# liangxuy/ReGenNet

Measured on AMD Instinct MI355X. Metric: sampled motions/sec, higher is better.
Workload: dtype bf16 MFMA operands, fp32 accumulate/LayerNorm/softmax, for 990 of 1000 steps; fp16 MFMA operands for the next 8; split-bf16 (x3) for the last 2; 1 GPU; ntu: [B=256/GPU,56,6,60] online/concat/no_cond L8 d512, 1000-step DDPM, Philox noise, hipGraph=on; batch_per_gpu=256, global_batch=256, denoiser_evals_per_motion=1000, parallelism=batch-shard x1

## Files before the change

regennet_amd/csrc/rgn_layers.hip:

```cpp
#include "rgn_internal.h"
#include "rgn_device.h"
#include "rgn_tail.h"
#include "rgn_sampler.h"

#include <hip/hip_runtime.h>

#include <cmath>
#include <type_traits>
#include <utility>

namespace rgn {

#ifndef RGN_LY_ST_AUX
#define RGN_LY_ST_AUX 16
#endif

constexpr int LY_NTH = 512, LY_KB = 4096;
constexpr int LY_X = 0, LY_Y = 64 * 1024, LY_EXCH = LY_Y, LY_RED = 128 * 1024, LY_REDF = 2 * 8 * 64, LY_VEC = LY_RED + 2 * LY_REDF * 4, LY_VECW = 640,
              LY_LDS = 160 * 1024;
constexpr int LY_PF = LY_VEC + 8 * LY_VECW * 4;
static_assert(LY_PF + 8 * 256 <= LY_LDS, "LDS map");
enum { V_BO = 0, V_G1 = 64, V_G2 = 128, V_B2 = 192, V_SPV = 256, V_BF1 = 320 , V_BF2 = 448, V_G3 = 512, V_B3 = 576 };
constexpr int LY_RDA = 6;
constexpr int LY_RDM = 8;
struct LYT {
    static constexpr int MT = 2, NT = 2, NW = 8, R = 64, RD = LY_RDM, KB = LY_KB, RED = LY_RED, REDF = LY_REDF;
};

#ifdef RGN_LY_STAMPS
__device__ long long g_ly_st[1024][16];
#define RGN_LYT(i)                                                                                   \
    {                                                                                                \
        __builtin_amdgcn_sched_barrier(0);                                                           \
        if (threadIdx.x == 0 && blockIdx.x < 1024 && l == RGN_LY_STAMPS) g_ly_st[blockIdx.x][i] = __builtin_readcyclecounter(); \
        __builtin_amdgcn_sched_barrier(0);                                                           \
    }
#define RGN_LYS(i)                                                                                   \
    {                                                                                                \
        __builtin_amdgcn_sched_barrier(0);                                                           \
        if (threadIdx.x == 0 && blockIdx.x < 1024 && it == 1) g_ly_st[blockIdx.x][i] = __builtin_readcyclecounter(); \
        __builtin_amdgcn_sched_barrier(0);                                                           \
    }
#else
#define RGN_LYT(i)
#define RGN_LYS(i)
#endif

constexpr int LY_XLD = 356, LY_TILE = 0, LY_XIMG = 92160, LY_NKX = 11;
static_assert(64 * LY_XLD * 4 <= LY_XIMG && LY_XIMG + LY_NKX * 4096 <= LY_LDS, "step boundary LDS map");

template <bool STEPS, bool GUIDED = false, bool F16 = false, bool INPAINT = false>
__global__ __launch_bounds__(LY_NTH, 2) void k_layers(LayersArgs g) {
    static_assert(STEPS || !GUIDED, "guidance inside the launch needs the step boundary");
    static_assert(STEPS || !INPAINT, "in-painting (rgn_set_inpainting) belongs to the step boundary");
    using OP = OpFmt<F16>;
    using op_t = typename OP::t;
    using op8 = typename OP::v8;
    using op4 = typename OP::v4;
    extern __shared__ __attribute__((aligned(16))) char smem[];
    const int tid = threadIdx.x, lane = tid & 63;
    const int wave = __builtin_amdgcn_readfirstlane(tid >> 6);
    const int wn = wave & 3, hg = wave >> 2;
    const int l31 = lane & 31, kh = lane >> 5;
    const int b = xcd_affine(blockIdx.x, gridDim.x), Tq = g.Tq;
    const size_t row0 = (size_t)b * Tq;
#ifdef RGN_LY_PRIO
    if (wave >= 4) __builtin_amdgcn_s_setprio(RGN_LY_PRIO);
#endif
    float* vec = reinterpret_cast<float*>(smem + LY_VEC) + wave * LY_VECW;
    const int lane16 = lane * 16;
    tile_dma_in(smem + LY_X, g.h, g.rows, row0, Tq, lane, wave);
    const int first_step = (g.stepvec || STEPS) ? *g.d_step : 0;
    const TailLane tl = tail_lane<LYT>(smem, lane, wave);
    static_assert(LY_X == 0, "a_off addresses the image at byte 0");
    int a_off[2], a_offy[2];
    tail_a_off(a_off, lane);
    tail_a_off(a_offy, a_off, LY_Y);
    using Pass = TailPass;
    op8 wf[LY_RDM][2];
    const float qs2 = g.qscale * 1.44269504088896340736f;

    f32x4 qb[4];
    float vb1;
    auto load_qbias = [&](const float* bqkv, int r) {
        const float* bq = bqkv + (2 * r + hg) * 128 + wn * 32;
#pragma unroll
        for (int i4 = 0; i4 < 4; ++i4) qb[i4] = *reinterpret_cast<const f32x4*>(bq + 8 * i4 + 4 * kh);
        vb1 = bq[1024 + l31];
    };

    wait_vmcnt<0>();
    __builtin_amdgcn_s_barrier();
    load_qbias(g.lw[0].bqkv, 0);

    const int nit = STEPS ? g.steps : 1;
    auto out_proj = [&](f32x16 (&acc)[2][2], int wv) {
#pragma unroll
        for (int a2 = 0; a2 < 2; ++a2)
#pragma unroll
            for (int b2 = 0; b2 < 2; ++b2)
#pragma unroll
                for (int i = 0; i < 16; ++i) acc[a2][b2][i] = 0.f;
        if (wv < 6) {
            const int cb0 = 2 * wv;
            const Pass p_out{__builtin_amdgcn_make_buffer_rsrc(const_cast<__bf16*>(g.Wout) + (size_t)cb0 * 1024, 0, (16 * g.nb_out - cb0) * 2048, 0x00020000), LY_NKX * 2048, 0};
#pragma unroll
            for (int s2 = 0; s2 < LY_RDM - 1; ++s2) tail_load_g<OP, LYT>(wf, tl, p_out, s2, s2);
            tail_gemm<OP, LYT, 32, false, 0>(acc, wf, tl, a_off, p_out, p_out);
        }
    };
    for (int it = 0; it < nit; ++it) {
    const int step = first_step - it;
    for (int pass = 0; pass < (GUIDED ? 2 : 1); ++pass) {
    if (GUIDED && pass == 1) {
        f32x16 accp[2][2];
        int wave_p = wave, lane_p = lane, b_p = b;
        asm volatile("" : "+s"(wave_p), "+s"(b_p));
        asm volatile("" : "+v"(lane_p));
        out_proj(accp, wave_p);
        if (wave_p < 6) {
            float* pk = g.park + ((size_t)b_p * 6 + wave_p) * 4096 + lane_p * 4;
#pragma unroll
            for (int nt = 0; nt < 2; ++nt)
#pragma unroll
                for (int mt = 0; mt < 2; ++mt)
#pragma unroll
                    for (int i4 = 0; i4 < 4; ++i4)
                        *reinterpret_cast<f32x4*>(pk + ((nt * 2 + mt) * 4 + i4) * 256) = f32x4{accp[nt][mt][4 * i4], accp[nt][mt][4 * i4 + 1], accp[nt][mt][4 * i4 + 2], accp[nt][mt][4 * i4 + 3]};
        }
        __builtin_amdgcn_s_barrier();
        tile_dma_in<16>(smem + LY_X, g.h, g.rows, g.half + (size_t)b_p * Tq, Tq, lane_p, wave_p);
        wait_vmcnt<0>();
        __builtin_amdgcn_s_barrier();
    }
    for (int l = 0; l < g.L; ++l) {
        const LayerWts& w = g.lw[l];
        RGN_LYT(0)
        op4 attk[2][2][4];
        float bo_r = 0.f;
        {
            struct PassA { __amdgpu_buffer_rsrc_t rs; };
            auto qrs = [&](int r) {
                const int blk = (2 * r + hg) * 4 + wn;
                return __builtin_amdgcn_make_buffer_rsrc(const_cast<__bf16*>(w.Wqkv) + (size_t)blk * 1024, 0, 3 * 512 * 512 * 2 - blk * 2048, 0x00020000);
            };
            const PassA pa[2] = {{qrs(0)}, {qrs(1)}};
            op8 wq[LY_RDA][3];
            auto load_ga = [&](const PassA& ps, int hs, int slot) {
                int soff;
                asm volatile("s_mov_b32 %0, %1" : "=s"(soff) : "i"(frag_granule(hs, 48 * 2048)));
#pragma unroll
                for (int t = 0; t < 3; ++t)
                    wq[slot][t] = __builtin_bit_cast(op8, __builtin_amdgcn_raw_buffer_load_b128(ps.rs, lane16, soff + t * (16 * 2048), 0));
            };
            constexpr int AH = LY_RDA - 1;
#pragma unroll
            for (int s = 0; s < AH; ++s) load_ga(pa[0], s, s);
#pragma unroll
            for (int r = 0; r < 2; ++r) {
                const int head = 2 * r + hg;
                f32x16 acc[2][3];
#pragma unroll
                for (int ta = 0; ta < 2; ++ta)
#pragma unroll
                    for (int i4 = 0; i4 < 4; ++i4)
#pragma unroll
                        for (int e = 0; e < 4; ++e) {
                            acc[ta][0][4 * i4 + e] = qb[i4][e];
                            acc[ta][1][4 * i4 + e] = 0.f;
                            acc[ta][2][4 * i4 + e] = vb1;
                        }
                __builtin_amdgcn_sched_barrier(0);
                {
                    op8 af[2];
#pragma unroll
                    for (int ta = 0; ta < 2; ++ta) af[ta] = *reinterpret_cast<const op8*>(smem + a_off[0] + ta * 2048);
#pragma unroll
                    for (int hs = 0; hs < 32; ++hs) {
                        op8 afn[2];
#pragma unroll
                        for (int ta = 0; ta < 2; ++ta) {
                            afn[ta] = af[ta];
                            if (hs + 1 < 32) afn[ta] = *reinterpret_cast<const op8*>(smem + ((hs + 1) >> 1) * LY_KB + a_off[(hs + 1) & 1] + ta * 2048);
                        }
                        if (hs + AH < 32) load_ga(pa[r], hs + AH, (32 * r + hs + AH) % LY_RDA);
                        else if (r == 0) load_ga(pa[1], hs + AH - 32, (32 * r + hs + AH) % LY_RDA);
                        if (hs + AH < 32 || r == 0) {
                            if (hs < AH) wait_vmcnt<3 * AH + 5>();
                            else wait_vmcnt<3 * AH>();
                        }
                        const int slot = (32 * r + hs) % LY_RDA;
#pragma unroll
                        for (int t = 0; t < 3; ++t)
#pragma unroll
                            for (int ta = 0; ta < 2; ++ta) {
                                if (t < 2) acc[ta][t] = OP::mfma(wq[slot][t], af[ta], acc[ta][t]);
                                else acc[ta][t] = OP::mfma(af[ta], wq[slot][t], acc[ta][t]);
                            }
#pragma unroll
                        for (int ta = 0; ta < 2; ++ta) af[ta] = afn[ta];
                    }
                }
                __builtin_amdgcn_sched_barrier(0);
                RGN_LYT(1 + 3 * r)
                op8 qh[2][2], kf[2][2], vh[2][2];
#pragma unroll
                for (int ta = 0; ta < 2; ++ta)
#pragma unroll
                    for (int sl = 0; sl < 2; ++sl)
#pragma unroll
                        for (int j = 0; j < 8; ++j) {
                            const int i = 8 * sl + j;
                            qh[ta][sl][j] = (op_t)acc[ta][0][i];
                            kf[ta][sl][j] = (op_t)acc[ta][1][i];
                            vh[ta][sl][j] = (op_t)acc[ta][2][i];
                        }
                if (r == 0) load_qbias(w.bqkv, 1);
                else bo_r = w.bo[64 * wave + lane];
                f32x16 st[3];
#pragma unroll
                for (int tl = 0; tl < 3; ++tl) {
                    const int kj = tl >> 1, qtile = tl ? 1 : 0;
#pragma unroll
                    for (int i = 0; i < 16; ++i) st[tl][i] = 0.f;
#pragma unroll
                    for (int sl = 0; sl < 2; ++sl) st[tl] = OP::mfma(kf[kj][sl], qh[qtile][sl], st[tl]);
                }
                f32x4* sred = reinterpret_cast<f32x4*>(smem + LY_EXCH);
#pragma unroll
                for (int tl = 0; tl < 3; ++tl)
#pragma unroll
                    for (int i4 = 0; i4 < 4; ++i4) {
                        const f32x4 v = {st[tl][4 * i4], st[tl][4 * i4 + 1], st[tl][4 * i4 + 2], st[tl][4 * i4 + 3]};
                        sred[(((hg * 3 + tl) * 4 + wn) * 4 + i4) * 64 + lane] = v;
                    }
                if (r == 0) { RGN_LYT(12) }
                wait_lgkmcnt<0>();
                __builtin_amdgcn_s_barrier();
                if (r == 0) { RGN_LYT(13) }
                {
                    const int kg = lane & 3, qi = lane >> 2, qt = qi >> 3, ql = 8 * wn + (qi & 7), Q = 32 * qt + ql;
                    const int kj = kg >> 1, sl = kg & 1;
                    const bool live = !(qt == 0 && kj == 1);
                    const int tl = live ? qt + kj : 0;
                    const char* ex = smem + LY_EXCH + ((hg * 3 + tl) * 4 * 4 + 2 * sl) * 1024 + ql * 16;
                    f32x4 sv[4];
#pragma unroll
                    for (int a2 = 0; a2 < 2; ++a2)
#pragma unroll
                        for (int h2 = 0; h2 < 2; ++h2) {
                            f32x4 v = *reinterpret_cast<const f32x4*>(ex + a2 * 1024 + h2 * 512);
#pragma unroll
                            for (int ww = 1; ww < 4; ++ww) {
                                const f32x4 u = *reinterpret_cast<const f32x4*>(ex + ww * 4096 + a2 * 1024 + h2 * 512);
#pragma unroll
                                for (int e = 0; e < 4; ++e) v[e] += u[e];
                            }
                            sv[2 * a2 + h2] = v;
                        }
                    int xlim = live ? (Q < Tq - 1 ? Q : Tq - 1) - 32 * kj - 16 * sl : -1;
                    asm volatile("" : "+v"(xlim));
                    float mx = -INFINITY;
#pragma unroll
                    for (int c4 = 0; c4 < 4; ++c4)
#pragma unroll
                        for (int e = 0; e < 4; ++e) {
                            sv[c4][e] = (4 * c4 + e <= xlim) ? sv[c4][e] : -INFINITY;
                            mx = fmaxf(mx, sv[c4][e]);
                        }
                    mx = fmaxf(mx, __builtin_bit_cast(float, __builtin_amdgcn_mov_dpp(__builtin_bit_cast(int, mx), 0xB1, 0xf, 0xf, true)));
                    mx = fmaxf(mx, __builtin_bit_cast(float, __builtin_amdgcn_mov_dpp(__builtin_bit_cast(int, mx), 0x4E, 0xf, 0xf, true)));
                    float sum = 0.f;
                    const float nmx = -mx * qs2;
#pragma unroll
                    for (int c4 = 0; c4 < 4; ++c4)
#pragma unroll
                        for (int e = 0; e < 4; ++e) {
                            sv[c4][e] = __builtin_amdgcn_exp2f(__builtin_fmaf(sv[c4][e], qs2, nmx));
                            sum += sv[c4][e];
                        }
                    sum += __builtin_bit_cast(float, __builtin_amdgcn_mov_dpp(__builtin_bit_cast(int, sum), 0xB1, 0xf, 0xf, true));
                    sum += __builtin_bit_cast(float, __builtin_amdgcn_mov_dpp(__builtin_bit_cast(int, sum), 0x4E, 0xf, 0xf, true));
                    const float inv = 1.0f / sum;
                    if (live) {
#pragma unroll
                        for (int h2 = 0; h2 < 2; ++h2) {
                            op8 pp;
#pragma unroll
                            for (int e = 0; e < 4; ++e) {
                                pp[e] = (op_t)(sv[h2][e] * inv);
                                pp[4 + e] = (op_t)(sv[2 + h2][e] * inv);
                            }
                            *reinterpret_cast<op8*>(smem + LY_EXCH + (((hg * 3 + tl) * 4 + 0) * 4 + sl) * 1024 + (h2 * 32 + ql) * 16) = pp;
                        }
                    }
                }
                if (r == 0) { RGN_LYT(14) }
                wait_lgkmcnt<0>();
                __builtin_amdgcn_s_barrier();
                if (r == 0) { RGN_LYT(15) }
#pragma unroll
                for (int qtile = 0; qtile < 2; ++qtile) {
                    f32x16 oa;
#pragma unroll
                    for (int i = 0; i < 16; ++i) oa[i] = 0.f;
#pragma unroll
                    for (int tl = qtile; tl <= 2 * qtile; ++tl) {
                        const int kj = tl >> 1;
#pragma unroll
                        for (int sl = 0; sl < 2; ++sl) {
                            const op8 ph = *reinterpret_cast<const op8*>(smem + LY_EXCH + (((hg * 3 + tl) * 4 + 0) * 4 + sl) * 1024 + lane * 16);
                            oa = OP::mfma(vh[kj][sl], ph, oa);
                        }
                    }
#pragma unroll
                    for (int i4 = 0; i4 < 4; ++i4)
#pragma unroll
                        for (int e = 0; e < 4; ++e) attk[r][qtile][i4][e] = (op_t)oa[4 * i4 + e];
                }
                RGN_LYT(2 + 3 * r)
                wait_lgkmcnt<0>();
                __builtin_amdgcn_s_barrier();
                RGN_LYT(3 + 3 * r)
            }
        }
        const Pass p_wo{tail_wrs(w.Wo, 2 * wave, 512 * 512 * 2), 16 * 2048, 0}, p_w1a{tail_wrs(w.W1, 2 * wave, 1024 * 512 * 2), 32 * 2048, 0},
            p_w1b{tail_wrs(w.W1, 16 + 2 * wave, 1024 * 512 * 2), 32 * 2048, 0}, p_w2a{tail_wrs(w.W2, 2 * wave, 512 * 1024 * 2), 16 * 2048, 0},
            p_w2b{p_w2a.rs, 16 * 2048, 32};
        vec[V_BO + lane] = bo_r;
#pragma unroll
        for (int s = 0; s < LY_RDM - 1; ++s) tail_load_g<OP, LYT>(wf, tl, p_wo, s, s);
        int cw = 64 * wave + lane;
        asm volatile("" : "+v"(cw));
        float vv[12];
        {
            const float* src[9] = {w.bo, w.g1, w.g2, w.b2, w.bf1, w.bf1 + 512, w.bf2, w.g3, w.b3};
            vv[1] = src[1][cw]; vv[2] = src[2][cw]; vv[3] = src[3][cw];
            vv[4] = w.b1[cw] + (g.stepvec ? g.stepvec[(size_t)step * g.ldstep + (size_t)l * 512 + cw] : 0.f) +
                    (g.pervec ? g.pervec[((size_t)b + (size_t)pass * g.B) * g.ldper + (size_t)l * 512 + cw] : 0.f);
            vv[5] = src[4][cw]; vv[6] = src[5][cw]; vv[7] = src[6][cw]; vv[8] = src[7][cw]; vv[9] = src[8][cw];
        }
        asm volatile("" ::: "memory");
#pragma unroll
        for (int r = 0; r < 2; ++r)
#pragma unroll
            for (int qtile = 0; qtile < 2; ++qtile)
#pragma unroll
                for (int i4 = 0; i4 < 4; ++i4)
                    *reinterpret_cast<op4*>(smem + LY_Y + ((2 * r + hg) * 4 + wn) * LY_KB + (32 * qtile + l31) * 64 + img_slot(i4, tl.swz) + 8 * kh) = attk[r][qtile][i4];
        wait_lgkmcnt<0>();
        __builtin_amdgcn_s_barrier();
        f32x16 acc[2][2];
        tail_init_bias<LYT>(acc, tl, vec + V_BO);
        RGN_LYT(7)
        tail_gemm<OP, LYT, 32, true, 11>(acc, wf, tl, a_offy, p_wo, p_w1a);
        RGN_LYT(8)
        vec[V_G1 + lane] = vv[1]; vec[V_G2 + lane] = vv[2]; vec[V_B2 + lane] = vv[3]; vec[V_SPV + lane] = vv[4];
        vec[V_BF1 + lane] = vv[5]; vec[V_BF1 + 64 + lane] = vv[6]; vec[V_BF2 + lane] = vv[7]; vec[V_G3 + lane] = vv[8]; vec[V_B3 + lane] = vv[9];
        tail_add_resid<OP, LYT>(acc, tl, LY_X);
        tail_layernorm<LYT, 0>(acc, tl, vec + V_G1, tail_rowvec(tl, vec + V_SPV));
        tail_layernorm<LYT, 1>(acc, tl, vec + V_G2, tail_rowvec(tl, vec + V_B2));
        tail_store_img<OP, LYT>(acc, tl, LY_X);
        wait_lgkmcnt<0>();
        __builtin_amdgcn_s_barrier();
        RGN_LYT(9)
        f32x16 acc2[2][2];
        tail_ffn<OP, LYT>(acc2, wf, tl, a_off, a_offy, LY_Y, p_w1a, p_w1b, p_w2a, p_w2b, vec + V_BF1, vec + V_BF2);
        load_qbias(g.lw[l + 1 < g.L ? l + 1 : 0].bqkv, 0);
#ifndef RGN_LY_NO_PREFETCH
        if constexpr (STEPS) {
            if (l == g.L - 1) {
                const int nsl = (int)(gridDim.x >> 3) >= 32 ? 32 : ((int)(gridDim.x >> 3) > 0 ? (int)(gridDim.x >> 3) : 1);
                const int sl = (int)(blockIdx.x >> 3) % nsl;
                const int n_out = 16 * g.nb_out * 16, n_all = n_out + LY_NKX * 16 * 16;
                const unsigned pf_lds = (unsigned)(size_t)((RGN_AS3 char*)(smem + LY_PF)) + (unsigned)wave * 256u;
                for (int ln = sl + nsl * tid; ln < n_all; ln += nsl * LY_NTH) {
                    const char* pp = ln < n_out ? reinterpret_cast<const char*>(g.Wout) + (size_t)ln * 128 : reinterpret_cast<const char*>(g.Wx) + (size_t)(ln - n_out) * 128;
                    int m0_keep;
                    asm volatile("s_mov_b32 %0, m0\n\ts_mov_b32 m0, %2\n\ts_nop 0\n\tglobal_load_lds_dword %1, off\n\ts_mov_b32 m0, %0" : "=&s"(m0_keep) : "v"(pp), "s"(pf_lds) : "memory");
                }
            }
        }
#endif
        RGN_LYT(10)
        tail_add_resid<OP, LYT>(acc2, tl, LY_X);
        tail_layernorm<LYT, 0>(acc2, tl, vec + V_G3, tail_rowvec(tl, vec + V_B3));
        tail_store_img<OP, LYT>(acc2, tl, LY_X);
        wait_lgkmcnt<0>();
        __builtin_amdgcn_s_barrier();
        RGN_LYT(11)
    }
    }
    if constexpr (STEPS) {
        int lane_s = lane, wave_s = wave, b_s = b;
        asm volatile("" : "+v"(lane_s));
        asm volatile("" : "+s"(wave_s), "+s"(b_s));
        const int l31_s = lane_s & 31, kh_s = lane_s >> 5;
        const size_t row0_s = (size_t)b_s * Tq;
        auto col4s = [&](int nt, int i4) { return 32 * nt + 8 * i4 + 4 * kh_s; };
        RGN_LYS(12)
        const SampleParams sp = *g.sp;
        const StepCoef k = g.tab[step];
        const int T = Tq, gb = g.s0 + b_s;
        const float gscale = GUIDED ? g.scale[gb] : 0.f;
        const __amdgpu_buffer_rsrc_t park_rs = __builtin_amdgcn_make_buffer_rsrc(GUIDED ? g.park + ((size_t)b_s * 6 + (wave_s < 6 ? wave_s : 0)) * 4096 : nullptr, 0, 4096 * 4, 0x00020000);
        f32x16 acc[2][2];
        out_proj(acc, wave_s);
        __builtin_amdgcn_s_barrier();
        float* tile = reinterpret_cast<float*>(smem + LY_TILE);
#pragma unroll
        for (int nt = 0; nt < 2; ++nt)
#pragma unroll
            for (int i4 = 0; i4 < 4; ++i4) {
                const int n = 64 * wave_s + col4s(nt, i4);
                if (n < 352) {
                    f32x4 bb = {0.f, 0.f, 0.f, 0.f};
                    if (n < g.F) bb = *reinterpret_cast<const f32x4*>(g.bout + n);
#pragma unroll
                    for (int mt = 0; mt < 2; ++mt) {
                        f32x4 v = {acc[nt][mt][4 * i4] + bb[0], acc[nt][mt][4 * i4 + 1] + bb[1], acc[nt][mt][4 * i4 + 2] + bb[2], acc[nt][mt][4 * i4 + 3] + bb[3]};
                        if constexpr (GUIDED) {
                            const f32x4 cc = __builtin_bit_cast(f32x4, __builtin_amdgcn_raw_buffer_load_b128(park_rs, (lane_s * 4 + ((nt * 2 + mt) * 4 + i4) * 256) * 4, 0, 16));
#pragma unroll
                            for (int e = 0; e < 4; ++e) v[e] = guide(cc[e] + bb[e], v[e], gscale);
                        }
                        *reinterpret_cast<f32x4*>(tile + (32 * mt + l31_s) * LY_XLD + n) = v;
                    }
                }
            }
        const Pass p_wx{__builtin_amdgcn_make_buffer_rsrc(const_cast<__bf16*>(g.Wx) + (size_t)(2 * wave_s) * 1024, 0, (LY_NKX * 16 - 2 * wave_s) * 2048, 0x00020000), 16 * 2048, 0};
#pragma unroll
        for (int s2 = 0; s2 < LY_RDM - 1; ++s2) tail_load_g<OP, LYT>(wf, tl, p_wx, s2, s2);
        op4 c0v[2][2][4];
#pragma unroll
        for (int mt = 0; mt < 2; ++mt) {
            const int r = 32 * mt + l31_s, rr = r < T ? r : T - 1;
#pragma unroll
            for (int nt = 0; nt < 2; ++nt)
#pragma unroll
                for (int i4 = 0; i4 < 4; ++i4)
                    c0v[nt][mt][i4] = *reinterpret_cast<const op4*>(g.c0 + (row0_s + rr) * 512 + 64 * wave_s + col4s(nt, i4));
        }
        op4 c0u[GUIDED ? 2 : 1][2][4];
        if constexpr (GUIDED) {
#pragma unroll
            for (int mt = 0; mt < 2; ++mt) {
                const int r = 32 * mt + l31_s, rr = r < T ? r : T - 1;
#pragma unroll
                for (int nt = 0; nt < 2; ++nt)
#pragma unroll
                    for (int i4 = 0; i4 < 4; ++i4)
                        c0u[nt][mt][i4] = *reinterpret_cast<const op4*>(g.c0 + ((size_t)g.half + row0_s + rr) * 512 + 64 * wave_s + col4s(nt, i4));
            }
        }
        wait_lgkmcnt<0>();
        __builtin_amdgcn_s_barrier();
        RGN_LYS(13)
        {
            const int t = lane_s;
            const bool valid = t < T;
            const size_t FT = (size_t)g.F * T;
            const int bn = noise_motion(sp, gb);
            char* ximg = smem + LY_XIMG;
            const int q = lane_s & 3, tq = t - q;
            const bool run4 = valid && (tq & 3) == 0 && tq + 3 < T;
            const bool quads = !sp.noise && !g.no_quads && __all(run4 || tq >= T);
            float xpre[LY_NKX][4];
#pragma unroll
            for (int i2 = 0; i2 < LY_NKX; ++i2)
#pragma unroll
                for (int j = 0; j < 4; ++j) {
                    const int f = 4 * (wave_s + 8 * i2) + j;
                    xpre[i2][j] = (valid && f < g.F) ? sp.x[(size_t)gb * FT + (size_t)f * T + t] : 0.f;
                }
            const int ximg_lane = img_run(lane_s, wave_s >> 1, wave_s & 1);
            constexpr int LY_IPD = GUIDED ? 1 : 2;
            unsigned char mpre[INPAINT ? LY_NKX : 1][4];
            float ipre[INPAINT ? LY_NKX : 1][4];
            const InpaintRsrc irs = inpaint_rsrc(sp, INPAINT ? (size_t)gb * FT : 0, INPAINT ? FT : 0);
            auto inp_request = [&](auto IG) __attribute__((always_inline)) {
                constexpr int ig = decltype(IG)::value;
                if constexpr (INPAINT && ig < LY_NKX) {
#pragma unroll
                    for (int j = 0; j < 4; ++j) inpaint_load(irs, t, (4 * (wave_s + 8 * ig) + j) * T, mpre[ig][j], ipre[ig][j]);
                    asm volatile("" ::: "memory");
                }
            };
            static_for<LY_IPD>([&](auto IG) __attribute__((always_inline)) { inp_request(IG); });
            auto update4 = [&](int i2, int fg, const float (&eps_in)[4], const float (&xv)[4]) {
                op4 nvb;
#pragma unroll
                for (int j = 0; j < 4; ++j) nvb[j] = (op_t)0.f;
                if (valid && 4 * fg < g.F) {
                    const f32x4 x04 = *reinterpret_cast<const f32x4*>(tile + lane_s * LY_XLD + 4 * fg);
#pragma unroll
                    for (int j = 0; j < 4; ++j) {
                        const int f = 4 * fg + j;
                        unsigned char im = 0;
                        float iv = 0.f;
                        if constexpr (INPAINT) { im = mpre[i2][j]; iv = ipre[i2][j]; }
                        const float x0 = pred_x0<INPAINT>(x04[j], im, iv, sp.clip);
                        const size_t o = (size_t)gb * FT + (size_t)f * T + t;
                        if (sp.x0_out) sp.x0_out[o] = x0;
                        const float nv = sampler_next(k, sp.sampler, x0, xv[j], quad_or_step_eps(quads, eps_in[j], sp, step, g.B, FT, bn, f, T, t));
                        sp.x[o] = nv;
                        nvb[j] = (op_t)nv;
                    }
                }
                *reinterpret_cast<op4*>(ximg + i2 * 4096 + ximg_lane) = nvb;
            };
            static_for<LY_NKX>([&](auto IT) __attribute__((always_inline)) {
                constexpr int i2 = decltype(IT)::value;
                const int fg = wave_s + 8 * i2;
                inp_request(std::integral_constant<int, i2 + LY_IPD>{});
                float eps4[4] = {0.f, 0.f, 0.f, 0.f};
                if (quads) quad_normals(sp, step, bn, fg, q, tq, eps4);
                update4(i2, fg, eps4, xpre[i2]);
            });
        }
        wait_lgkmcnt<0>();
        __builtin_amdgcn_s_barrier();
        RGN_LYS(14)
#pragma unroll
        for (int a2 = 0; a2 < 2; ++a2)
#pragma unroll
            for (int b2 = 0; b2 < 2; ++b2)
#pragma unroll
                for (int i = 0; i < 16; ++i) acc[a2][b2][i] = 0.f;
        {
            int a_offx[2] = {a_off[0] + LY_XIMG, a_off[1] + LY_XIMG};
            tail_gemm<OP, LYT, 2 * LY_NKX, false, 8 + 16>(acc, wf, tl, a_offx, p_wx, p_wx);
        }
        if constexpr (GUIDED) {
            __builtin_amdgcn_s_barrier();
#pragma unroll
            for (int nt = 0; nt < 2; ++nt)
#pragma unroll
                for (int i4 = 0; i4 < 4; ++i4)
#pragma unroll
                    for (int mt = 0; mt < 2; ++mt) {
                        op4 hh;
#pragma unroll
                        for (int e = 0; e < 4; ++e) hh[e] = (op_t)(acc[nt][mt][4 * i4 + e] + (float)c0u[nt][mt][i4][e]);
                        *tail_img_run<OP, LYT>(tl, LY_Y, nt, i4, mt) = hh;
                    }
        }
#pragma unroll
        for (int nt = 0; nt < 2; ++nt)
#pragma unroll
            for (int mt = 0; mt < 2; ++mt)
#pragma unroll
                for (int i4 = 0; i4 < 4; ++i4)
#pragma unroll
                    for (int e = 0; e < 4; ++e) acc[nt][mt][4 * i4 + e] += (float)c0v[nt][mt][i4][e];
        tail_store_img<OP, LYT>(acc, tl, LY_X);
        wait_lgkmcnt<0>();
        __builtin_amdgcn_s_barrier();
        if constexpr (GUIDED) {
            const __amdgpu_buffer_rsrc_t u_rs = __builtin_amdgcn_make_buffer_rsrc(g.out, 0, (int)((size_t)g.rows * 512 * 2), 0x00020000);
            const int r16 = lane_s >> 2, c = lane_s & 3;
#pragma unroll
            for (int j = 0; j < 8; ++j) {
                const int p = wave_s * 8 + j, blk = p >> 2, r = (p & 3) * 16 + r16;
                if (r < T) {
                    const int off = blk * LY_KB + r * 64 + ((c ^ ((r >> 2) & 3)) << 4);
                    __builtin_amdgcn_raw_buffer_store_b128(*reinterpret_cast<const u32x4*>(smem + LY_Y + off), u_rs,
                                                           (int)((((size_t)blk * g.rows + g.half + row0_s + r) * 32 + c * 8) * 2), 0, RGN_LY_ST_AUX);
                }
            }
        }
        RGN_LYS(15)
    }
    }
    {
        const __amdgpu_buffer_rsrc_t o_rs = __builtin_amdgcn_make_buffer_rsrc(g.out, 0, (int)((size_t)g.rows * 512 * 2), 0x00020000);
        const int r16 = lane >> 2, c = lane & 3;
#pragma unroll
        for (int j = 0; j < 8; ++j) {
            const int p = wave * 8 + j, blk = p >> 2, r = (p & 3) * 16 + r16;
            if (r < Tq) {
                const int off = blk * LY_KB + img_chunk(r, c);
                __builtin_amdgcn_raw_buffer_store_b128(*reinterpret_cast<const u32x4*>(smem + LY_X + off), o_rs,
                                                       (int)(plane_chunk(g.rows, row0 + r, blk, c) * 2), 0, RGN_LY_ST_AUX);
            }
        }
    }
    if constexpr (STEPS) {
        if (tid == 0) step_ticket(g.d_stepw + 4, (int)gridDim.x, g.d_stepw, first_step - g.steps);
    }
}

#ifdef RGN_LY_STAMPS
void ly_stamps_read(long long* out) { (void)hipMemcpyFromSymbol(out, HIP_SYMBOL(g_ly_st), sizeof(long long) * 1024 * 16); }
#endif

bool layers_supported(int d, int ff, int H, int Tq, int L) { return d == 512 && ff == 1024 && H == 4 && Tq >= 1 && Tq <= 64 && L >= 1 && L <= LY_MAXL; }
bool layers_steps_supported(int d, int F, int Kpx) { return d == 512 && F % 4 == 0 && F <= 352 && Kpx == 32 * LY_NKX; }
constexpr bool layers_form_exists(bool steps, bool guided, bool inpaint) { return steps || !(guided || inpaint); }
template <class Fn>
static hipError_t layers_form(bool steps, bool guided, bool f16, bool inpaint, Fn fn) {
    return dispatch_bools([&](auto S, auto G, auto H, auto I) {
        if constexpr (layers_form_exists(decltype(S)::value, decltype(G)::value, decltype(I)::value))
            return fn(k_layers<decltype(S)::value, decltype(G)::value, decltype(H)::value, decltype(I)::value>);
        else
            return hipErrorInvalidValue;
    }, steps, guided, f16, inpaint);
}
hipError_t configure_layers() {
    hipError_t e = hipSuccess;
    for (int m = 0; m < 16 && e == hipSuccess; ++m)
        if (layers_form_exists(m & 1, m & 2, m & 8))
            e = layers_form(m & 1, m & 2, m & 4, m & 8, [](auto kern) { return hipFuncSetAttribute(reinterpret_cast<const void*>(kern), hipFuncAttributeMaxDynamicSharedMemorySize, LY_LDS); });
    return e;
}
hipError_t launch_layers(const LayersArgs& g, hipStream_t s, bool inpaint) {
    const bool steps = g.steps > 0;
    return layers_form(steps, steps && g.scale, g.f16 != 0, inpaint, [&](auto kern) {
        hipLaunchKernelGGL(kern, dim3(g.Bm), dim3(LY_NTH), LY_LDS, s, g);
        return hipGetLastError();
    });
}

}
```

regennet_amd/csrc/rgn_tail.h:

```cpp
#pragma once
#include "rgn_device.h"

namespace rgn {
namespace {

struct TailLane {
    char* smem;
    int lane16, wave, kh, swz;
    int img_base;
    int red_base;
    int red_base2;
};
template <class C>
__device__ __forceinline__ TailLane tail_lane(char* smem, int lane, int wave) {
    const int l31 = lane & 31, kh = lane >> 5;
    int img_base = (C::NT * wave) * C::KB + l31 * 64 + 8 * kh;
    asm volatile("" : "+v"(img_base));
    int red_base = C::RED + 4 * l31;
    asm volatile("" : "+v"(red_base));
    int red_base2 = red_base + 128 * kh;
    asm volatile("" : "+v"(red_base2));
    return TailLane{smem, lane * 16, wave, kh, img_swz(l31), img_base, red_base, red_base2};
}

__device__ __forceinline__ void tail_a_off(int (&a)[2], int lane) {
    const int l31 = lane & 31, kh = lane >> 5;
#pragma unroll
    for (int ks = 0; ks < 2; ++ks) a[ks] = img_frag(l31, ks, kh);
}
__device__ __forceinline__ void tail_a_off(int (&a)[2], const int (&a0)[2], int img) {
#pragma unroll
    for (int ks = 0; ks < 2; ++ks) a[ks] = a0[ks] + img;
}
__device__ __forceinline__ int tail_col4(const TailLane& t, int nt, int i4) { return 32 * nt + 8 * i4 + 4 * t.kh; }
template <class OP, class C>
__device__ __forceinline__ typename OP::v4* tail_img_run(const TailLane& t, int img, int nt, int i4, int mt) {
    return reinterpret_cast<typename OP::v4*>(t.smem + (img + t.img_base + img_slot(i4, t.swz)) + (nt * C::KB + mt * 2048));
}

struct TailPass { __amdgpu_buffer_rsrc_t rs; int kstride, hs0; };
__device__ __forceinline__ __amdgpu_buffer_rsrc_t tail_wrs(const __bf16* W, int cb0, int bytes) {
    return __builtin_amdgcn_make_buffer_rsrc(const_cast<__bf16*>(W) + (size_t)cb0 * 1024, 0, bytes - cb0 * 2048, 0x00020000);
}
template <class OP, class C>
__device__ __forceinline__ void tail_load_g(typename OP::v8 (&wf)[C::RD][C::NT], const TailLane& t, const TailPass& ps, int hs_rel, int slot) {
    const int hs = ps.hs0 + hs_rel;
    int soff;
    asm volatile("s_mov_b32 %0, %1" : "=s"(soff) : "i"(frag_granule(hs, ps.kstride)));
#pragma unroll
    for (int nt = 0; nt < C::NT; ++nt)
        wf[slot][nt] = __builtin_bit_cast(typename OP::v8, __builtin_amdgcn_raw_buffer_load_b128(ps.rs, t.lane16, soff + nt * 2048, 0));
}
template <class OP, class C, int NG, bool CH, int EX>
__device__ __forceinline__ void tail_gemm(f32x16 (&acc)[C::NT][C::MT], typename OP::v8 (&wf)[C::RD][C::NT], const TailLane& t, const int (&aoff)[2],
                                          const TailPass& cur, const TailPass& nxt) {
    using op8 = typename OP::v8;
    constexpr int MT = C::MT, NT = C::NT, RD = C::RD, AH = RD - 1;
    __builtin_amdgcn_sched_barrier(0);
    op8 af[MT];
#pragma unroll
    for (int mt = 0; mt < MT; ++mt) af[mt] = *reinterpret_cast<const op8*>(t.smem + aoff[0] + mt * 2048);
#pragma unroll
    for (int hs = 0; hs < NG; ++hs) {
        op8 afn[MT];
#pragma unroll
        for (int mt = 0; mt < MT; ++mt) {
            afn[mt] = af[mt];
            if (hs + 1 < NG) afn[mt] = *reinterpret_cast<const op8*>(t.smem + ((hs + 1) >> 1) * C::KB + aoff[(hs + 1) & 1] + mt * 2048);
        }
        if (hs + AH < NG) tail_load_g<OP, C>(wf, t, cur, hs + AH, (hs + AH) % RD);
        else if (CH) tail_load_g<OP, C>(wf, t, nxt, hs + AH - NG, (hs + AH) % RD);
        if (hs + AH < NG || CH) {
            if (hs < AH) wait_vmcnt<NT * AH + EX>();
            else wait_vmcnt<NT * AH>();
        }
#pragma unroll
        for (int nt = 0; nt < NT; ++nt)
#pragma unroll
            for (int mt = 0; mt < MT; ++mt) acc[nt][mt] = OP::mfma(wf[hs % RD][nt], af[mt], acc[nt][mt]);
#pragma unroll
        for (int mt = 0; mt < MT; ++mt) af[mt] = afn[mt];
    }
    __builtin_amdgcn_sched_barrier(0);
}

template <class C>
__device__ __forceinline__ void tail_init_bias(f32x16 (&acc)[C::NT][C::MT], const TailLane& t, const float* bias) {
#pragma unroll
    for (int nt = 0; nt < C::NT; ++nt)
#pragma unroll
        for (int i4 = 0; i4 < 4; ++i4) {
            const f32x4 b = *reinterpret_cast<const f32x4*>(bias + tail_col4(t, nt, i4));
#pragma unroll
            for (int mt = 0; mt < C::MT; ++mt)
#pragma unroll
                for (int e = 0; e < 4; ++e) acc[nt][mt][4 * i4 + e] = b[e];
        }
}
template <class C, int SLOT, class Shift>
__device__ __forceinline__ void tail_layernorm(f32x16 (&acc)[C::NT][C::MT], const TailLane& t, const float* gam, Shift shift) {
    constexpr int MT = C::MT, NT = C::NT, NW = C::NW, R = C::R;
    static_assert(MT == 2, "the two half_swaps hand over exactly two row tiles");
    const char* buf = t.smem + t.red_base + SLOT * C::REDF * 4;
    const char* buf2 = t.smem + t.red_base2 + SLOT * C::REDF * 4;
    const float invn = 1.0f / 512.f;
#pragma unroll
    for (int mt = 0; mt < MT; ++mt) {
        f32x2 s2 = f32x2{0.f, 0.f}, q2 = f32x2{0.f, 0.f};
#pragma unroll
        for (int nt = 0; nt < NT; ++nt)
#pragma unroll
            for (int i = 0; i < 16; i += 2) {
                const f32x2 v = f32x2{acc[nt][mt][i], acc[nt][mt][i + 1]};
                s2 += v;
                q2 = __builtin_elementwise_fma(v, v, q2);
            }
        float s = s2[0] + s2[1], q = q2[0] + q2[1];
        half_swap(s, q);
        *reinterpret_cast<float*>(const_cast<char*>(buf) + (t.kh * (NW * R) + t.wave * R + 32 * mt) * 4) = s + q;
    }
    wait_lgkmcnt<0>();
    __builtin_amdgcn_s_barrier();
    f32x2 rs[MT], nm[MT];
    {
        float p[2][NW];
#pragma unroll
        for (int st = 0; st < 2; ++st)
#pragma unroll
            for (int w = 0; w < NW; ++w) p[st][w] = *reinterpret_cast<const float*>(buf2 + (st * (NW * R) + w * R) * 4);
#pragma unroll
        for (int st = 0; st < 2; ++st)
#pragma unroll
            for (int d = 1; d < NW; d *= 2)
#pragma unroll
                for (int w = 0; w < NW; w += 2 * d) p[st][w] += p[st][w + d];
        const float mean = p[0][0] * invn;
        const float var = __builtin_fmaxf(p[1][0] * invn - mean * mean, 0.f);
        float r0 = __builtin_amdgcn_rsqf(var + 1e-5f), n0 = -mean * r0;
        float r1 = r0, n1 = n0;
        asm volatile("" : "+v"(r1), "+v"(n1));
        half_swap(r0, r1);
        half_swap(n0, n1);
        rs[0] = f32x2{r0, r0}; rs[1] = f32x2{r1, r1};
        nm[0] = f32x2{n0, n0}; nm[1] = f32x2{n1, n1};
    }
#pragma unroll
    for (int nt = 0; nt < NT; ++nt) {
        f32x4 ga[4], sh[4][MT];
#pragma unroll
        for (int i4 = 0; i4 < 4; ++i4) {
            ga[i4] = *reinterpret_cast<const f32x4*>(gam + tail_col4(t, nt, i4));
#pragma unroll
            for (int mt = 0; mt < MT; ++mt) sh[i4][mt] = shift(nt, i4, mt);
        }
#pragma unroll
        for (int i4 = 0; i4 < 4; ++i4)
#pragma unroll
            for (int mt = 0; mt < MT; ++mt)
#pragma unroll
                for (int e = 0; e < 4; e += 2) {
                    const f32x2 v = __builtin_elementwise_fma(f32x2{acc[nt][mt][4 * i4 + e], acc[nt][mt][4 * i4 + e + 1]}, rs[mt], nm[mt]);
                    const f32x2 o = __builtin_elementwise_fma(v, f32x2{ga[i4][e], ga[i4][e + 1]}, f32x2{sh[i4][mt][e], sh[i4][mt][e + 1]});
                    acc[nt][mt][4 * i4 + e] = o[0];
                    acc[nt][mt][4 * i4 + e + 1] = o[1];
                }
    }
}
__device__ __forceinline__ auto tail_rowvec(const TailLane& t, const float* v) {
    return [kh = t.kh, v](int nt, int i4, int) { return *reinterpret_cast<const f32x4*>(v + 32 * nt + 8 * i4 + 4 * kh); };
}

template <class OP, class C>
__device__ __forceinline__ void tail_store_img(const f32x16 (&acc)[C::NT][C::MT], const TailLane& t, int img) {
#pragma unroll
    for (int nt = 0; nt < C::NT; ++nt)
#pragma unroll
        for (int i4 = 0; i4 < 4; ++i4)
#pragma unroll
            for (int mt = 0; mt < C::MT; ++mt) {
                typename OP::v4 h;
#pragma unroll
                for (int e = 0; e < 4; ++e) h[e] = (typename OP::t)acc[nt][mt][4 * i4 + e];
                *tail_img_run<OP, C>(t, img, nt, i4, mt) = h;
            }
}
template <class OP, class C>
__device__ __forceinline__ void tail_add_resid(f32x16 (&acc)[C::NT][C::MT], const TailLane& t, int img) {
    typename OP::v4 r[C::NT][C::MT][4];
#pragma unroll
    for (int nt = 0; nt < C::NT; ++nt)
#pragma unroll
        for (int mt = 0; mt < C::MT; ++mt)
#pragma unroll
            for (int i4 = 0; i4 < 4; ++i4) r[nt][mt][i4] = *tail_img_run<OP, C>(t, img, nt, i4, mt);
#pragma unroll
    for (int nt = 0; nt < C::NT; ++nt)
#pragma unroll
        for (int mt = 0; mt < C::MT; ++mt)
#pragma unroll
            for (int i4 = 0; i4 < 4; ++i4)
#pragma unroll
                for (int e = 0; e < 4; ++e) acc[nt][mt][4 * i4 + e] += (float)r[nt][mt][i4][e];
}
template <class C>
__device__ __forceinline__ void tail_gelu(f32x16 (&acc)[C::NT][C::MT]) {
#pragma unroll
    for (int nt = 0; nt < C::NT; ++nt)
#pragma unroll
        for (int mt = 0; mt < C::MT; ++mt)
#pragma unroll
            for (int i = 0; i < 16; i += 2) {
                const f32x2 gl = gelu2_p13(f32x2{acc[nt][mt][i], acc[nt][mt][i + 1]});
                acc[nt][mt][i] = gl[0];
                acc[nt][mt][i + 1] = gl[1];
            }
}

template <class OP, class C>
__device__ __forceinline__ void tail_ffn(f32x16 (&acc2)[C::NT][C::MT], typename OP::v8 (&wf)[C::RD][C::NT], const TailLane& t, const int (&a_in)[2],
                                         const int (&a_hid)[2], int hid, const TailPass& w1a, const TailPass& w1b, const TailPass& w2a, const TailPass& w2b,
                                         const float* bf1, const float* bf2) {
    f32x16 acc[C::NT][C::MT];
    tail_init_bias<C>(acc2, t, bf2);
#pragma unroll
    for (int c = 0; c < 2; ++c) {
        tail_init_bias<C>(acc, t, bf1 + 32 * C::NT * c);
        tail_gemm<OP, C, 32, true, 0>(acc, wf, t, a_in, c ? w1b : w1a, c ? w2b : w2a);
        tail_gelu<C>(acc);
        if (c == 1) __builtin_amdgcn_s_barrier();
        tail_store_img<OP, C>(acc, t, hid);
        wait_lgkmcnt<0>();
        __builtin_amdgcn_s_barrier();
        if (c == 0) tail_gemm<OP, C, 32, true, 0>(acc2, wf, t, a_hid, w2a, w1b);
        else tail_gemm<OP, C, 32, false, 0>(acc2, wf, t, a_hid, w2b, w2b);
    }
}

}
}
```

Baseline: 464.0 motions/s.

## Restructure tail GEMM A-fragment prefetch and stagger block start phases

The tail GEMM inner loop now keeps row tile 0 in a double-buffered register pair and reloads row tile 1 into a single register right after its MFMAs. Explicit sched_group_barrier hints interleave the LDS reads with the MFMA group. The aim is to cut VGPR pressure from the old afn copy and to hide LDS latency behind matrix ops. Separately, persistent multi-step blocks now sleep a slot-dependent number of cycles before the step loop, staggering groups of blocks so they do not contend for weights or memory in lockstep. This adds a small fixed startup delay.

```diff
diff --git a/regennet_amd/csrc/rgn_layers.hip b/regennet_amd/csrc/rgn_layers.hip
--- a/regennet_amd/csrc/rgn_layers.hip
+++ b/regennet_amd/csrc/rgn_layers.hip
@@ -11,6 +11,9 @@
 
 namespace rgn {
 
+#ifndef RGN_LY_DEPHASE
+#define RGN_LY_DEPHASE 28
+#endif
 #ifndef RGN_LY_ST_AUX
 #define RGN_LY_ST_AUX 16
 #endif
@@ -109,6 +112,12 @@
             tail_gemm<OP, LYT, 32, false, 0>(acc, wf, tl, a_off, p_out, p_out);
         }
     };
+#if RGN_LY_DEPHASE
+    if (STEPS && nit >= 64) {
+        const int slot = (blockIdx.x >> 3) & 3;
+        for (int i = 0; i < slot * RGN_LY_DEPHASE; ++i) __builtin_amdgcn_s_sleep(16);
+    }
+#endif
     for (int it = 0; it < nit; ++it) {
     const int step = first_step - it;
     for (int pass = 0; pass < (GUIDED ? 2 : 1); ++pass) {
diff --git a/regennet_amd/csrc/rgn_tail.h b/regennet_amd/csrc/rgn_tail.h
--- a/regennet_amd/csrc/rgn_tail.h
+++ b/regennet_amd/csrc/rgn_tail.h
@@ -56,30 +56,33 @@
                                           const TailPass& cur, const TailPass& nxt) {
     using op8 = typename OP::v8;
     constexpr int MT = C::MT, NT = C::NT, RD = C::RD, AH = RD - 1;
+    static_assert(MT == 2, "row tile 0 alternates between two fragment registers, row tile 1 rotates in one");
     __builtin_amdgcn_sched_barrier(0);
-    op8 af[MT];
-#pragma unroll
-    for (int mt = 0; mt < MT; ++mt) af[mt] = *reinterpret_cast<const op8*>(t.smem + aoff[0] + mt * 2048);
+    op8 a0[2], a1;
+    a0[0] = *reinterpret_cast<const op8*>(t.smem + aoff[0]);
+    a1 = *reinterpret_cast<const op8*>(t.smem + aoff[0] + 2048);
+    __builtin_amdgcn_sched_barrier(0);
 #pragma unroll
     for (int hs = 0; hs < NG; ++hs) {
-        op8 afn[MT];
-#pragma unroll
-        for (int mt = 0; mt < MT; ++mt) {
-            afn[mt] = af[mt];
-            if (hs + 1 < NG) afn[mt] = *reinterpret_cast<const op8*>(t.smem + ((hs + 1) >> 1) * C::KB + aoff[(hs + 1) & 1] + mt * 2048);
-        }
         if (hs + AH < NG) tail_load_g<OP, C>(wf, t, cur, hs + AH, (hs + AH) % RD);
         else if (CH) tail_load_g<OP, C>(wf, t, nxt, hs + AH - NG, (hs + AH) % RD);
         if (hs + AH < NG || CH) {
             if (hs < AH) wait_vmcnt<NT * AH + EX>();
             else wait_vmcnt<NT * AH>();
         }
-#pragma unroll
-        for (int nt = 0; nt < NT; ++nt)
-#pragma unroll
-            for (int mt = 0; mt < MT; ++mt) acc[nt][mt] = OP::mfma(wf[hs % RD][nt], af[mt], acc[nt][mt]);
-#pragma unroll
-        for (int mt = 0; mt < MT; ++mt) af[mt] = afn[mt];
+        if (hs + 1 < NG) {
+            a0[(hs + 1) & 1] = *reinterpret_cast<const op8*>(t.smem + ((hs + 1) >> 1) * C::KB + aoff[(hs + 1) & 1]);
+            __builtin_amdgcn_sched_group_barrier(0x100, 1, 0);
+        }
+#pragma unroll
+        for (int nt = 0; nt < NT; ++nt) acc[nt][0] = OP::mfma(wf[hs % RD][nt], a0[hs & 1], acc[nt][0]);
+#pragma unroll
+        for (int nt = 0; nt < NT; ++nt) acc[nt][1] = OP::mfma(wf[hs % RD][nt], a1, acc[nt][1]);
+        __builtin_amdgcn_sched_group_barrier(0x8, MT * NT, 0);
+        if (hs + 1 < NG) {
+            a1 = *reinterpret_cast<const op8*>(t.smem + ((hs + 1) >> 1) * C::KB + aoff[(hs + 1) & 1] + 2048);
+            __builtin_amdgcn_sched_group_barrier(0x100, 1, 0);
+        }
     }
     __builtin_amdgcn_sched_barrier(0);
 }
```

Result: no change. 461.7 motions/s (-0.5%).
